# TimoLassmann/tagdust

Measured on AMD Instinct MI355X. Metric: reads/s (150 bp, 8-barcode arch), higher is better.
Workload: dtype f32

## Files before the change

include/tagdust_hip.h:

```cpp
#ifndef TAGDUST_HIP_H
#define TAGDUST_HIP_H

#include <stddef.h>
#include <stdint.h>

#ifdef __cplusplus
extern "C" {
#endif

#define TD_OK   0
#define TD_FAIL 1

#define TD_MAX_SEGMENTS 64
#define TD_MAX_HMMS     127
#define TD_LOGSUM_SIZE  16000

#define TD_MODE_GET_LABEL 1
#define TD_MODE_GET_PROB  4
#define TD_MODE_ARCH_COMP 5
#define TD_MODE_RNA_DUST  6

#define TD_EXTRACT_SUCCESS                    0
#define TD_EXTRACT_FAIL_ARCHITECTURE_MISMATCH 1
#define TD_EXTRACT_FAIL_READ_TOO_SHORT        2
// ... 39 lines not shown
	int32_t read_type;
	int32_t barcode;
	int32_t fingerprint;
} td_read_result;

int  td_ctx_create(int device, td_ctx** out);
void td_ctx_destroy(td_ctx* ctx);
const char* td_last_error(const td_ctx* ctx);

const float* td_logsum_table(void);

int td_model_upload(td_ctx* ctx, const td_model_desc* model);
int td_set_option(td_ctx* ctx, const char* name, int32_t value);
int td_get_option(td_ctx* ctx, const char* name, int32_t* value);
int64_t td_spec_source(const td_model_desc* model, char* buf, int64_t cap);
int td_spec_prune_info(const td_model_desc* model, int32_t lcap, float* tab, float* z, int32_t* n_seg, int32_t* sfx_first);
int td_spec_restart_info(const td_model_desc* model, int32_t lcap, float* tab, int32_t* restart);
#define TD_PROBE_READS     256
#define TD_PROBE_THRESHOLD 3.0f
#define TD_PROBE_MINLEN    16
#define TD_PROBE_DUST      100
#define TD_PROBE_WIN_START 2
#define TD_PROBE_WIN_END   34
int64_t td_spec_probe(const td_model_desc* model, uint8_t* codes, int64_t cap, int64_t* offs);
void td_spec_probe_params(float* threshold, int32_t* minlen, int32_t* dust, int32_t* matchstart, int32_t* matchend);
int td_spec_wait(td_ctx* ctx);
int td_set_artifacts(td_ctx* ctx, const uint8_t* string, const int32_t* s_index, int32_t n_seq,
                     int32_t filter_error, int32_t n_threads);
int td_set_window(td_ctx* ctx, int32_t matchstart, int32_t matchend);
int td_set_batch_window(td_ctx* ctx, int64_t first_read, int64_t total_reads);
// ... 35 lines not shown
```

tagdust_amd/csrc/td_api.hip:

```cpp
#include <math.h>
#include <stdarg.h>
#include <stdlib.h>
#include <string.h>
#include <time.h>
#include <unistd.h>

#include <mutex>
#include <thread>

#include "../../include/tagdust_model.h"
#include "td_ctx.h"
#include "td_rnadust.h"
#include "td_stats.h"

static float g_logsum[TD_LOGSUM_SIZE];
static bool g_logsum_ready = false;
static std::string g_create_error;

static void init_logsum_host()
{
	if (g_logsum_ready) return;
	for (int i = 0; i < TD_LOGSUM_SIZE; i++) g_logsum[i] = (float)log(1.0 + exp((double)-i / (double)1000.0f));
	g_logsum_ready = true;
}
// ... 233 lines not shown
	if (spec_model_uploaded(c) != TD_OK) return TD_FAIL;
	c->have_model = true;
	return TD_OK;
}

extern "C" int td_set_option(td_ctx* c, const char* name, int32_t value)
{
	if (!c || !name) return TD_FAIL;
	if (!strcmp(name, "specialize")) {
		c->spec.specialize = value != 0;
		return TD_OK;
	}
	if (!strcmp(name, "poison_workspace")) { c->poison = value != 0; return TD_OK; }
	if (!strcmp(name, "async_compile")) { c->spec.async_compile = value != 0; return TD_OK; }
	if (!strcmp(name, "spec_probe")) { c->spec.probe = value != 0; return TD_OK; }
	if (!strcmp(name, "compact_egress")) { c->compact_egress = value != 0; return TD_OK; }
	if (!strcmp(name, "stable_input")) {
		if (tickets_outstanding(c)) return fail(c, "td_set_option: stable_input cannot change while tickets are outstanding");
		c->stable_input = value != 0;
		return TD_OK;
	}
	if (!strcmp(name, "length_classes_enabled")) { c->length_classes = value != 0; return TD_OK; }
	if (!strcmp(name, "debug_wait")) { c->debug_wait = value != 0; return TD_OK; }
	if (!strcmp(name, "spec_lsum_limit")) { c->spec.lsum_limit = value > 0 ? (double)value : 1.0e6; return TD_OK; }
	if (!strcmp(name, "rle_cap")) {
		if (value < 0 || value > 127) return fail(c, "td_set_option: rle_cap must be 0 (default) .. 127");
		c->rle_cap_forced = value;
		return TD_OK;
	}
	if (!strcmp(name, "host_threads")) {
// ... 11 lines not shown
		if (tickets_outstanding(c)) return fail(c, "td_set_option: pipeline_depth cannot change while tickets are outstanding");
		c->pipeline_depth = value; c->next_slot = 0;
		return TD_OK;
	}
	return fail(c, "td_set_option: unknown option %s", name);
}

extern "C" int td_get_option(td_ctx* c, const char* name, int32_t* value)
{
	if (!c || !name || !value) return TD_FAIL;
	if (!strcmp(name, "specialize")) { *value = c->spec.specialize; return TD_OK; }
	if (!strcmp(name, "spec_lsum_clamped")) { *value = c->spec.ready && !c->spec.oob; return TD_OK; }
	if (!strcmp(name, "pipeline_depth")) { *value = c->pipeline_depth; return TD_OK; }
	if (!strcmp(name, "async_compile")) { *value = c->spec.async_compile; return TD_OK; }
	if (!strcmp(name, "spec_probe")) { *value = c->spec.probe; return TD_OK; }
	if (!strcmp(name, "spec_state")) { *value = spec_state_now(c); return TD_OK; }
	if (!strcmp(name, "spec_batches_generic")) { *value = c->spec.batches_generic; return TD_OK; }
	if (!strcmp(name, "spec_compiles_started")) { *value = td_spec_compiles_started(); return TD_OK; }
	if (!strcmp(name, "spec_probe_us")) { *value = c->spec.probe_us; return TD_OK; }
	if (!strcmp(name, "host_threads")) { *value = c->host_threads; return TD_OK; }
	if (!strcmp(name, "artifacts_active")) { *value = c->art_n > 0; return TD_OK; }
	if (!strcmp(name, "dust")) { *value = c->dust; return TD_OK; }
	if (!strcmp(name, "length_classes")) { *value = c->slots[c->last_slot].n_big; return TD_OK; }
	if (!strcmp(name, "overlap_decode")) { *value = c->overlap; return TD_OK; }
	if (!strcmp(name, "compact_egress")) { *value = c->compact_egress; return TD_OK; }
	if (!strcmp(name, "stable_input")) { *value = c->stable_input; return TD_OK; }
	if (!strcmp(name, "length_classes_enabled")) { *value = c->length_classes; return TD_OK; }
	if (!strcmp(name, "hw_queues")) { *value = g_hwq_user ? g_hwq_user : (g_hwq_late ? 4 : 8); return TD_OK; }
	if (!strcmp(name, "hw_queues_late")) { *value = g_hwq_late ? 1 : 0; return TD_OK; }
	if (!strcmp(name, "prune_active")) {
// ... 854 lines not shown
```

tagdust_amd/csrc/td_ctx.h:

```cpp
#pragma once
#include <hip/hip_runtime.h>
#include <stdio.h>
#include <memory>
#include <string>
#include <vector>
#include "../../include/tagdust_hip.h"
#include "td_device.h"
#include "td_batch_plan.h"
#include "td_jit.h"
#include "td_stage.h"
#include "td_host_inner.h"
#include "td_census.h"
#include "td_molecules.h"

#define TD_HIDDEN __attribute__((visibility("hidden")))
#define TD_MAX_PIPELINE 4
#define TD_COUNTER_WORDS (TD_NUM_COUNTERS + TD_NUM_DIAG_COUNTERS)

struct TdRoute {
	hipStream_t cs = nullptr;
	hipStream_t aux = nullptr;
	hipStream_t fin = nullptr;
	int wsi = 0;
	bool pipelined = false;
// ... 96 lines not shown
};

struct SpecJob;
struct TdSpecState {
	int specialize = 1;
	bool ready = false;
	hipModule_t mod = nullptr;  hipFunction_t fn = nullptr;
	TdSpecPlan plan;
	bool oob = false;
	bool window = false;
	bool oob_unsafe = false;
	float maxabs = 0.0f;
	int block = 256, waves_per_cu = 8;
	int async_compile = 0;
	int probe = 1;
	int state = 0;
	int batches_generic = 0;
	int probe_us = 0;
	std::shared_ptr<SpecJob> job;
	int job_oob = 0, job_window = 0;
	std::vector<std::shared_ptr<SpecJob>> retired;
	std::string job_err;
	double lsum_limit = 1.0e6;
	int selfcheck_fail = 0;
	float* d_prune = nullptr;   int prune_lcap = 0, prune_stride = 0;
	bool prune_live = false;
};

TD_HIDDEN int default_host_threads();
struct td_ctx {
// ... 143 lines not shown
```

tagdust_amd/csrc/td_jit.h:

```cpp
#pragma once
#include <string>
#include <vector>
#include "../../include/tagdust_hip.h"
#include "td_device.h"

struct TdSpecKnobs {
	int block = 512;
	int min_waves = 4;
	int lsum_oob = 1;
	int rt_min = 16;
	int groupcols = 18;
	int groupcols_fwd = 12;
	int prune = 1;
	int prune_sfx = 1;
	int restart = -1;
	int firstseg = -1;
	int trie_sh = 2;
	int profile = 0;
	int prune_stats = -1;
	std::string extra_opts;
};
TdSpecKnobs td_spec_knobs(void);

#define TD_PRUNE_TABLES 16
#define TD_PRUNE_RESTART_MAX 4

struct TdSpecPlan {
	TdSpecKnobs k;
	int S = 0, H = 0, C = 0;
	std::vector<int> col_off, hmm_off;
	std::vector<int> group, group_f;
	std::vector<int> pure_last, drop_m;
	std::vector<int> bw_off;
	int64_t halves = 0;
	std::vector<int> rt, rt_b;
	std::vector<int> base;
// ... 19 lines not shown
```

tagdust_amd/csrc/td_jit.hip:

```cpp
#include <hip/hip_runtime.h>
#include <hip/hiprtc.h>
#include <math.h>
#include <stdio.h>
#include <string.h>
#include <stdlib.h>

#include <atomic>
#include <map>
#include <mutex>
#include <string>
#include <vector>

#include "../../include/tagdust_hip.h"
#include "td_device.h"
#include <unistd.h>
#include <sys/stat.h>
#include <sys/types.h>
#include "td_embedded_src.h"
#include "td_jit.h"

static std::string flit(float v)
{
	if (isinf(v)) return v < 0 ? "(-__builtin_inff())" : "__builtin_inff()";
	if (v != v) return "__builtin_nanf(\"\")";
// ... 9 lines not shown
	auto flag = [](const char* name, int unset) -> int { const char* e = getenv(name); return e ? atoi(e) != 0 : unset; };
	if (const int v = num("TD_SPEC_BLOCK", 0); v >= 64 && v <= 1024 && v % 64 == 0) k.block = v;
	if (const int v = num("TD_SPEC_MINWAVES", 0); v >= 1 && v <= 8) k.min_waves = v;
	if (const int v = num("TD_SPEC_GROUPCOLS", 0); v > 0) k.groupcols = v;
	k.groupcols_fwd = num("TD_SPEC_GROUPCOLS_FWD", k.groupcols_fwd);
	k.rt_min = num("TD_SPEC_RT_MIN", k.rt_min);
	k.trie_sh = num("TD_SPEC_TRIE_SH", k.trie_sh);
	k.profile = num("TD_SPEC_PROFILE", k.profile);
	k.lsum_oob = flag("TD_SPEC_LSUM_OOB", k.lsum_oob);
	k.prune = flag("TD_SPEC_PRUNE", k.prune);
	k.prune_sfx = flag("TD_SPEC_PRUNE_SFX", k.prune_sfx);
	k.restart = flag("TD_SPEC_RESTART", k.restart);
	k.firstseg = flag("TD_SPEC_FIRSTSEG", k.firstseg);
	k.prune_stats = flag("TD_SPEC_PRUNE_STATS", k.prune_stats);
	if (const char* e = getenv("TD_SPEC_EXTRA_OPTS")) k.extra_opts = e;
	return k;
}

namespace {
int pure_last(const td_model_desc* m, int j, int col_off)
{
	for (int f = 0; f < m->n_hmm[j]; f++) {
		const int q = col_off + f * m->n_col[j] + m->n_col[j] - 1;
		if (!(m->trans[q * 9 + 4] == -INFINITY) || !(m->trans[q * 9 + 3] == -INFINITY)) return 0;
	}
	return 1;
}

int rt_prefix(const td_model_desc* m, int j, int col_off, int* base , float* hi, float* lo, float* nv, int min_hmms)
{
	const int n = m->n_hmm[j], nc = m->n_col[j];
	if (n < min_hmms) return 0;
// ... 309 lines not shown

int td_spec_compile(const td_model_desc* m, const TdSpecPlan& p, int lsum_oob, int window, std::vector<char>& code, std::string& log,
                    uint64_t* key_out, bool key_only)
{
	const std::string src = td_spec_full_source(m, p, lsum_oob, window);
	std::vector<const char*> opts = { "--offload-arch=gfx950", "-O3", "-std=c++17", "-ffp-contract=off", "-fno-fast-math",
	                                  "-fno-slp-vectorize", "-mllvm", "-disable-machine-licm" };
	std::vector<std::string> extra;
	{
		std::string cur;
		for (const char* c = p.k.extra_opts.c_str();; c++) {
			if (*c == ' ' || *c == 0) { if (!cur.empty()) extra.push_back(cur); cur.clear(); if (!*c) break; }
			else cur += *c;
		}
	}
	for (const std::string& o : extra) opts.push_back(o.c_str());
	std::string keytext = src;
	for (const char* o : opts) keytext += std::string(" ") + o;
	{
		int major = 0, minor = 0, rt = 0;
		(void)hiprtcVersion(&major, &minor);
		(void)hipRuntimeGetVersion(&rt);
		keytext += " hiprtc " + std::to_string(major) + "." + std::to_string(minor) + " runtime " + std::to_string(rt);
	}
	const uint64_t key = fnv1a(keytext);
	if (key_out) *key_out = key;
	if (key_only) return TD_OK;
	std::string cache_file;
	const std::string dir = td_spec_cache_dir();
	if (!dir.empty()) {
		char name[64];
// ... 78 lines not shown

extern "C" int td_spec_restart_info(const td_model_desc* model, int32_t lcap, float* tab, int32_t* restart)
{
	if (!model || lcap < 1) return -1;
	const TdSpecPlan p = td_spec_plan(model, td_spec_knobs());
	if (restart) *restart = p.restart;
	if (tab) {
		std::vector<float> t;
		if (p.prune_segs > 0 || p.sfx_first < p.S) td_spec_prune_tables(model, p, lcap, lcap + 8, t);
		else t.assign((size_t)TD_PRUNE_TABLES * (size_t)(lcap + 8), -3.0e38f);
		memcpy(tab, t.data() + (size_t)8 * (size_t)(lcap + 8), (size_t)8 * (size_t)(lcap + 8) * sizeof(float));
	}
	return 0;
}

extern "C" int64_t td_spec_source(const td_model_desc* model, char* buf, int64_t cap)
{
	if (!model) return -1;
	const TdSpecPlan p = td_spec_plan(model, td_spec_knobs());
	const std::string src = td_spec_full_source(model, p, p.k.lsum_oob, 0);
	if (buf && cap > 0) {
		const size_t n = src.size() < (size_t)(cap - 1) ? src.size() : (size_t)(cap - 1);
		memcpy(buf, src.data(), n);
		buf[n] = '\0';
	}
	return (int64_t)src.size();
}
```

tagdust_amd/csrc/td_spec_host.hip:

```cpp
#include <stdlib.h>
#include <algorithm>
#include <cmath>
#include <condition_variable>
#include <map>
#include <mutex>
#include <thread>

#include "td_ctx.h"

struct SpecJob {
	uint64_t key = 0;
	ModelCopy model;
	TdSpecPlan plan;
	int lsum_oob = 0, window = 0;
	std::mutex mu;
	std::condition_variable cv;
	bool done = false;
	int rc = TD_FAIL;
	std::vector<char> code;
	std::string log;
	std::thread th;
	void run()
	{
		std::vector<char> out;
// ... 131 lines not shown
	pc.soa_a = d + o_outa; pc.soa_b = d + o_outb; pc.soa_stride = ol.soa_stride;
	pc.keep_a = ka.out_keep; pc.keep_b = sa.out_keep; pc.labels_a = ka.out_labels; pc.labels_b = sa.out_labels;
	pc.counters_a = cnt_a; pc.counters_b = cnt_b;
	pc.out = (int32_t*)(d + o_cmp);
	HIPCHK(c, td_probe_compare(pc, st));
	int32_t out[1 + 2 * (TD_PROBE_READS / TD_WAVE + 1)];
	HIPCHK(c, hipMemcpyAsync(out, d + o_cmp, sizeof out, hipMemcpyDeviceToHost, st));
	HIPCHK(c, hipStreamSynchronize(st));
	c->spec.prune_lcap = 0; c->spec.prune_live = false;
	v = ProbeVerdict();
	v.mismatches = out[0];
	for (int w = 0; w <= n_tiles && v.read < 0; w++) if (out[1 + 2 * w] >= 0) { v.read = out[1 + 2 * w]; v.field = out[2 + 2 * w]; }
	return TD_OK;
}

static int load_spec_kernel(td_ctx* c, int lsum_oob, int window = -1);
static int start_spec_job(td_ctx* c, int lsum_oob, int window);

static int install_spec_kernel(td_ctx* c, const std::vector<char>& code, uint64_t key, int lsum_oob, int window, bool background)
{
	TdSpecState& sp = c->spec;
	if (spec_unload(c) != TD_OK) return TD_FAIL;
	HIPCHK(c, hipModuleLoadData(&sp.mod, code.data()));
	HIPCHK(c, hipModuleGetFunction(&sp.fn, sp.mod, "td_spec_kernel"));
	{
		static const float g[] = { 0.0f, 0.0005f, 0.001f, 1.0f, 15.699f, 15.6999f, 15.7f, 15.7001f, 16.639f, 16.64f, 16.7f, 100.0f, 1.0e5f, 1.0e6f };
		std::vector<float> pairs;
		for (float base : { 0.0f, -3.25f, -700.0f }) {
			for (float d : g) { pairs.push_back(base); pairs.push_back(base - d); pairs.push_back(base - d); pairs.push_back(base); }
			pairs.push_back(base); pairs.push_back(-INFINITY); pairs.push_back(-INFINITY); pairs.push_back(base);
		}
		pairs.push_back(-INFINITY); pairs.push_back(-INFINITY);
		const int n_pairs = (int)(pairs.size() / 2);
		hipFunction_t chk = nullptr;
// ... 28 lines not shown
		ProbeVerdict v;
		bool known = false;
		{
			std::lock_guard<std::mutex> lk(g_probe_mu);
			auto it = g_probe_verdicts.find({ key, c->device });
			if (it != g_probe_verdicts.end()) { v = it->second; known = true; }
		}
		if (!known) {
			const double t0 = wall_ms();
			if (probe_spec_kernel(c, window, v) != TD_OK) return TD_FAIL;
			sp.probe_us = (int)((wall_ms() - t0) * 1000.0);
			std::lock_guard<std::mutex> lk(g_probe_mu);
			g_probe_verdicts[{ key, c->device }] = v;
		}
		if (v.mismatches != 0) {
			fprintf(stderr, "tagdust_hip: PROBE REJECTED the specialised kernel %016llx on device %d: %d of %d probe reads differ from the generic "
			        "kernel, first at read %d, field %s%s.  This context decodes with the generic kernel: correct, about ten times slower.\n",
			        (unsigned long long)key, c->device, v.mismatches, TD_PROBE_READS, v.read, probe_field_name(v.field), known ? " (verdict of an earlier load)" : "");
			if (spec_unload(c) != TD_OK) return TD_FAIL;
			sp.state = 4;
			return TD_OK;
		}
	}
	sp.ready = true; sp.window = window != 0; sp.oob = lsum_oob != 0;
	sp.state = 3;
	return TD_OK;
}

static int load_spec_kernel(td_ctx* c, int lsum_oob, int window)
{
	if (window < 0) window = c->match_len > 0;
	if (spec_unload(c) != TD_OK) return TD_FAIL;
	std::vector<char> code;
	std::string log;
	uint64_t key = 0;
	if (td_spec_compile(&c->model.d, c->spec.plan, lsum_oob, window, code, log, &key) != TD_OK) {
		c->spec.state = 5;
		return fail(c, "td_model_upload: specialised kernel did not compile: %.400s", log.c_str());
	}
	return install_spec_kernel(c, code, key, lsum_oob, window, false);
}

static int start_spec_job(td_ctx* c, int lsum_oob, int window)
{
	std::vector<char> none;
	std::string log;
	uint64_t key = 0;
	(void)td_spec_compile(&c->model.d, c->spec.plan, lsum_oob, window, none, log, &key, true);
	static std::once_flag at_exit_once;
	std::call_once(at_exit_once, [] { (void)atexit(wait_for_all_spec_jobs); });
	std::shared_ptr<SpecJob> job;
	{
		std::lock_guard<std::mutex> lk(g_jobs_mu);
		for (auto it = g_jobs.begin(); it != g_jobs.end();) { if (it->second.expired()) it = g_jobs.erase(it); else ++it; }
		auto it = g_jobs.find(key);
		if (it != g_jobs.end()) job = it->second.lock();
		if (!job) {
			job = std::make_shared<SpecJob>();
			job->key = key; job->model.assign(&c->model.d); job->plan = c->spec.plan; job->lsum_oob = lsum_oob; job->window = window;
			SpecJob* raw = job.get();
			job->th = std::thread([raw] { raw->run(); });
			g_jobs[key] = job;
		}
	}
	c->spec.job = job; c->spec.job_oob = lsum_oob; c->spec.job_window = window;
	c->spec.state = 1;
	return TD_OK;
}

int spec_handover(td_ctx* c, bool block)
{
	if (!c->spec.job) return c->spec.state == 5 && !c->spec.job_err.empty() ? fail(c, "%s", c->spec.job_err.c_str()) : TD_OK;
	if (!block && !c->spec.job->finished()) return TD_OK;
	c->spec.job->wait();
	const std::shared_ptr<SpecJob> job = std::move(c->spec.job);
	if (job->rc != TD_OK) {
		c->spec.state = 5;
		(void)fail(c, "td_model_upload: specialised kernel did not compile (background compile): %.400s", job->log.c_str());
		c->spec.job_err = c->err;
		return TD_FAIL;
	}
	c->spec.state = 2;
	HIPCHK(c, hipSetDevice(c->device));
	HIPCHK(c, sync_compute(c));
	return install_spec_kernel(c, job->code, job->key, c->spec.job_oob, c->spec.job_window, true);
}

extern "C" int td_spec_wait(td_ctx* c)
{
	if (!c) return TD_FAIL;
	while (c->spec.job) if (spec_handover(c, true) != TD_OK) return TD_FAIL;
	return spec_handover(c, false);
}

int spec_state_now(td_ctx* c) { return c->spec.job ? (c->spec.job->finished() ? 2 : 1) : c->spec.state; }
void spec_retire_jobs(td_ctx* c, bool wait)
{
	if (c->spec.job) { c->spec.retired.push_back(c->spec.job); c->spec.job.reset(); }
	if (wait) { for (auto& j : c->spec.retired) j->wait(); c->spec.retired.clear(); return; }
	for (size_t k = 0; k < c->spec.retired.size();) { if (c->spec.retired[k]->finished()) c->spec.retired.erase(c->spec.retired.begin() + (long)k); else k++; }
// ... 19 lines not shown

int spec_model_uploaded(td_ctx* c)
{
	TdSpecState& sp = c->spec;
	if (spec_unload(c) != TD_OK) return TD_FAIL;
	sp.prune_lcap = 0; sp.prune_live = false;
	sp.state = 0; sp.batches_generic = 0; sp.probe_us = 0;
	if (!sp.specialize) return TD_OK;
	const td_model_desc* m = &c->model.d;
	float mx = 0.0f;
	auto scan = [&](const float* v, size_t n) { for (size_t i = 0; i < n; i++) if (std::isfinite(v[i]) && fabsf(v[i]) > mx) mx = fabsf(v[i]); };
	scan(m->trans, (size_t)m->C * 9); scan(m->eM, (size_t)m->C * 5); scan(m->eI, (size_t)m->C * 5);
	scan(m->sM, m->C); scan(m->sI, m->C); scan(m->skip, m->S); scan(m->bg, 5);
	sp.maxabs = mx;
	sp.plan = td_spec_plan(m, td_spec_knobs());
	sp.block = sp.plan.k.block;
	const int wpb = sp.block / TD_WAVE;
	const int blocks_per_cu = std::min(2, std::max(1, 32 / wpb));
	sp.waves_per_cu = std::min(blocks_per_cu * wpb, 4 * sp.plan.k.min_waves);
	const int oob = sp.oob_unsafe ? 0 : sp.plan.k.lsum_oob;
	return sp.async_compile ? start_spec_job(c, oob, c->match_len > 0) : load_spec_kernel(c, oob);
}
```

tagdust_amd/csrc/td_spec_kernel.inc:

```

#ifndef TDS_BLOCK
#define TDS_BLOCK 512
#endif
#ifndef TDS_MIN_WAVES
#define TDS_MIN_WAVES 4
#endif
#define TDS_REG_H 32
#define TDS_WPB (TDS_BLOCK / TD_WAVE)
#define NEG_INF (-__builtin_inff())
#define DEV __device__ __forceinline__

#define MODE_GET_LABEL 1
#define MODE_ARCH_COMP 5
#define OUT_SUCCESS 0
#define OUT_ARCH_MISMATCH 1
#define OUT_TOO_SHORT 2
#define OUT_BAR_FINGER_NOT_FOUND 3
#define OUT_MATCHES_ARTIFACTS 5
#define OUT_LOW_COMPLEXITY 6
#define N_OUTCOME_SLOTS 8
#define TDS_DIAG(k) (N_OUTCOME_SLOTS + 256 + ((k) - 192))

#ifndef TDS_LSUM_OOB
#define TDS_LSUM_OOB 1
#endif
#if TDS_LSUM_OOB
#define TDS_TABLE_N 16640
#else
#define TDS_TABLE_N (TD_LOGSUM_LIVE + 4)
#endif
__shared__ float g_T[TDS_TABLE_N];

DEV float lsum(float a, float b)
{
#if TDS_LSUM_OOB
	const float t = __builtin_fabsf(a - b) * 4000.0f;
	int idx;
	asm("v_cvt_i32_f32 %0, %1" : "=v"(idx) : "v"(t));
	const float tv = *(const float*)((const char*)g_T + ((unsigned)idx & ~3u));
	return fmaxf(a, b) + tv;
#else
	const float mx = fmaxf(a, b);
	const float dc = fminf(mx - fminf(a, b), 15.7f);
	return mx + g_T[(int)(dc * 1000.0f)];
#endif
}

struct SV { float v; bool z; };
DEV SV sv(float v) { SV r; r.v = v; r.z = false; return r; }
DEV SV sv_none() { SV r; r.v = NEG_INF; r.z = true; return r; }
#define LIVE(v) ((v) != NEG_INF)
DEV SV addc(const SV a, const float c) { SV r; r.z = a.z || !LIVE(c); r.v = r.z ? NEG_INF : a.v + c; return r; }
DEV SV addv(const SV a, const float x) { SV r; r.z = a.z; r.v = a.z ? NEG_INF : a.v + x; return r; }
DEV SV subv(const SV a, const float x) { SV r; r.z = a.z; r.v = a.z ? NEG_INF : a.v - x; return r; }
DEV SV lsum(const SV a, const SV b) { if (a.z) return b; if (b.z) return a; return sv(lsum(a.v, b.v)); }

DEV void lsum2(SV& a0, const SV b0, SV& a1, const SV b1)
{
#if TDS_LSUM_OOB
	if (!a0.z && !b0.z && !a1.z && !b1.z) {
		const float t0 = __builtin_fabsf(a0.v - b0.v) * 4000.0f, t1 = __builtin_fabsf(a1.v - b1.v) * 4000.0f;
		int i0, i1;
		asm("v_cvt_i32_f32 %0, %1" : "=v"(i0) : "v"(t0));
		asm("v_cvt_i32_f32 %0, %1" : "=v"(i1) : "v"(t1));
		const float m0 = fmaxf(a0.v, b0.v), m1 = fmaxf(a1.v, b1.v);
		const float v0 = *(const float*)((const char*)g_T + ((unsigned)i0 & ~3u));
		const float v1 = *(const float*)((const char*)g_T + ((unsigned)i1 & ~3u));
		__builtin_amdgcn_sched_barrier(0);
		a0 = sv(m0 + v0);
		a1 = sv(m1 + v1);
		return;
	}
#endif
	a0 = lsum(a0, b0);
	a1 = lsum(a1, b1);
}

struct SI { float lo, hi; bool z; };
DEV SI si(float lo, float hi) { SI r; r.lo = lo; r.hi = hi; r.z = false; return r; }
DEV SI si(float v) { return si(v, v); }
DEV SI si_none() { SI r; r.lo = NEG_INF; r.hi = NEG_INF; r.z = true; return r; }
DEV SI addc(const SI a, const float c) { SI r; r.z = a.z || !LIVE(c); r.lo = r.z ? NEG_INF : a.lo + c; r.hi = r.z ? NEG_INF : a.hi + c; return r; }
DEV SI addv(const SI a, const float x) { SI r; r.z = a.z; r.lo = a.z ? NEG_INF : a.lo + x; r.hi = a.z ? NEG_INF : a.hi + x; return r; }
DEV float lsum_term(const float d)
{
#if TDS_LSUM_OOB
	const float t = d * 4000.0f;
	int idx;
	asm("v_cvt_i32_f32 %0, %1" : "=v"(idx) : "v"(t));
	return *(const float*)((const char*)g_T + ((unsigned)idx & ~3u));
#else
	return g_T[(int)(fminf(d, 15.7f) * 1000.0f)];
#endif
}
DEV SI lsum(const SI a, const SI b)
{
	if (a.z) return b;
	if (b.z) return a;
	const float dmin = fmaxf(fmaxf(a.lo - b.hi, b.lo - a.hi), 0.0f);
	const float dmax = fmaxf(a.hi - b.lo, b.hi - a.lo);
	return si(fmaxf(a.lo, b.lo) + lsum_term(dmax), fmaxf(a.hi, b.hi) + lsum_term(dmin));
}
DEV bool same(const SI a) { return a.lo == a.hi || (!(a.lo > NEG_INF) && !(a.hi > NEG_INF)); }

typedef float f32x4 __attribute__((ext_vector_type(4)));
// ... 355 lines not shown
#undef EM
}

template <int J, bool RT, int GC>
DEV void stair_dispatch(const int gc, const int fa, float (&Mlo)[kNCol[J]], float (&Mhi)[kNCol[J]], float (&Ilo)[kNCol[J]], float (&Ihi)[kNCol[J]],
                        const float Pn, const BaseMask& kc, const int c, const BaseMask& kx, const int xi)
{
	if constexpr (kNCol[J] > TDS_STAIR_STATIC_COLS) {
		stair_step<J, RT, -2>(gc, fa, Mlo, Mhi, Ilo, Ihi, Pn, kc, c, kx, xi);
	} else if constexpr (GC >= -1) {
		if (gc == GC) stair_step<J, RT, GC>(gc, fa, Mlo, Mhi, Ilo, Ihi, Pn, kc, c, kx, xi);
		else stair_dispatch<J, RT, GC - 1>(gc, fa, Mlo, Mhi, Ilo, Ihi, Pn, kc, c, kx, xi);
	}
}

template <int J, bool RT>
DEV void bwd_stair(const Wv& w, const uint8_t* __restrict__ codes, const float* __restrict__ P, const int fa, const int p_hi, const int p_lo)
{
	constexpr int NC = kNCol[J];
	constexpr int K = NC - 1;
	constexpr bool p_init = (J == TD_S - 1);
#define PBW(pos) (p_init ? (((pos) == w.len + 1) ? 0.0f : NEG_INF) : P[(pos) * TD_WAVE + w.lane])
	const float h = w.hb[(p_hi + 1) * TD_WAVE + w.lane];
	float Mlo[NC], Mhi[NC], Ilo[NC], Ihi[NC];
#pragma unroll
	for (int g = 0; g < NC; g++) { Mlo[g] = NEG_INF; Ilo[g] = NEG_INF; Mhi[g] = h; Ihi[g] = h; }
	int gc = K;
	int c = codes[(p_hi + 1) * TD_WAVE + w.lane];
	float Pn = PBW(p_hi + 1);
	int xi_n = codes[p_hi * TD_WAVE + w.lane];
	float Pi_n = PBW(p_hi);
	int i = p_hi;
// ... 21 lines not shown
	}
	close_check(p_hi - p_lo); close_check(p_hi - p_lo);
	if (gc >= 0) w.bad |= 32;
	if (TDS_PRUNE_STATS && w.lane == 0) {
		const int st = closed_at >= 0 ? closed_at : p_hi - p_lo;
		atomicAdd(&w.stats[TDS_DIAG(196)], (unsigned long long)st); atomicAdd(&w.stats[TDS_DIAG(197)], 1ull);
		atomicMax(&w.stats[TDS_DIAG(193)], (unsigned long long)st);
	}
	float* rs = w.rs + (int64_t)(kColOff[J] + fa * NC) * 2 * TD_WAVE + w.lane;
#pragma unroll
	for (int g = 0; g < NC; g++) { rs[(2 * g) * TD_WAVE] = Mlo[g]; rs[(2 * g + 1) * TD_WAVE] = Ilo[g]; }
#undef PBW
}

template <int J, int F>
DEV void bwd_stair_rest(const Wv& w, const uint8_t* __restrict__ codes, const float* __restrict__ P, const int p_hi, const int p_lo)
{
	if constexpr (F < kNHmm[J]) {
		bwd_stair<J, false>(w, codes, P, F, p_hi, p_lo);
		bwd_stair_rest<J, F + 1>(w, codes, P, p_hi, p_lo);
	}
}

#define TDS_BWD_BOUNDS(d, pos) { const int k_ = w.len - (pos); wc_q[d] = w.wc[k_ >= 1 ? k_ - 1 : 0]; if (skip_live) wd_q[d] = w.wd[k_ >= 0 ? k_ : 0]; }
#define TDS_BWD_STEP(SPILL_, WANT_CS_) \
		const int xi = xi_q[d_]; \
		const bool tailb = sfx_nb && i < w.sstopS; \
		const float Pi = tailb ? NEG_INF : Pi_q[d_]; \
		if (tailb) Pn = NEG_INF; \
		SV cs; cs.v = cs_q[d_]; cs.z = RT ? false : first; \
		{ \
// ... 170 lines not shown
DEV void fold_first_rest(const Wv& w, const int x1, const BaseMask& kx, const float Pi, SV& cs)
{
	if constexpr (F < kNHmm[J]) {
		fold_first_hmm<J, F, false>(w, F, x1, kx, Pi, cs);
		fold_first_rest<J, F + 1>(w, x1, kx, Pi, cs);
	}
}
template <int J>
DEV void bwd_fold_first(const Wv& w, const uint8_t* __restrict__ codes, const float* __restrict__ P, float* __restrict__ Cs)
{
	if (w.len < 1) return;
	const int x1 = codes[1 * TD_WAVE + w.lane];
	const BaseMask kx = mk_mask(x1);
	constexpr bool p_init = (J == TD_S - 1);
	const float Pi = p_init ? ((1 == w.len + 1) ? 0.0f : NEG_INF) : P[1 * TD_WAVE + w.lane];
	SV cs; cs.v = NEG_INF; cs.z = false;
	if constexpr (kRt[J] > 0) { for (int f = 0; f < kRt[J]; f++) fold_first_hmm<J, 0, true>(w, f, x1, kx, Pi, cs); }
	fold_first_rest<J, kRt[J]>(w, x1, kx, Pi, cs);
	Cs[1 * TD_WAVE + w.lane] = cs.v;
}

template <int J, int F0>
DEV void bwd_groups(const Wv& w, const uint8_t* __restrict__ codes, const float* __restrict__ P,
                    float* __restrict__ Cs, uint8_t* __restrict__ BW)
{
	if constexpr (TDS_RESTART && F0 == 0 && J < kPruneSegs) {
		if (w.rb_on) {
			const int p_lo = w.cutS + J * (w.rW + 1), p_hi = p_lo + w.rW;
			bwd_stair_bounds<J>(w, p_hi, p_hi);
			if constexpr (kRtB[J] > 0) { for (int f = 0; f < kRtB[J]; f++) bwd_stair<J, true>(w, codes, P, f, p_hi, p_lo); }
			bwd_stair_rest<J, kRtB[J]>(w, codes, P, p_hi, p_lo);
		}
	}
	if constexpr (F0 == 0 && kRt[J] > 0) {
		if constexpr (kTrieOn && J == 0) {
			for (int f0 = 0; f0 < kTrieNShare * kGroup[J]; f0 += kGroup[J]) bwd_group<J, kGroup[J], true, kTrieSH>(w, codes, P, Cs, BW, f0);
			for (int f0 = kTrieNShare * kGroup[J]; f0 < kRt[J]; f0 += kGroup[J]) bwd_group<J, kGroup[J], true>(w, codes, P, Cs, BW, f0);
		} else {
			for (int f0 = 0; f0 < kRt[J]; f0 += kGroup[J]) bwd_group<J, kGroup[J], true>(w, codes, P, Cs, BW, f0);
		}
		bwd_groups<J, kRt[J]>(w, codes, P, Cs, BW);
	} else if constexpr (F0 < kNHmm[J]) {
		constexpr int NF = cmin(kGroup[J], kNHmm[J] - F0);
		bwd_group<J, NF, false>(w, codes, P, Cs, BW, F0);
		bwd_groups<J, F0 + NF>(w, codes, P, Cs, BW);
	} else if constexpr (kTrieOn && J == 0) {
		bwd_fold_first<J>(w, codes, P, Cs);
	}
}

template <int J>
DEV void bwd_segments(const Wv& w, const uint8_t* __restrict__ codes, float* __restrict__ SB, int rowlen,
                      uint8_t* __restrict__ BW)
{
	if constexpr (J >= 0) {
		bwd_groups<J, 0>(w, codes, SB + (int64_t)(J + 1) * rowlen, SB + (int64_t)J * rowlen, BW);
		if (TDS_PROFILE == 2 && J < 8) { const long long t_ = (long long)__builtin_readcyclecounter(); if (w.lane == 0) atomicAdd(&w.stats[TDS_DIAG(208 + J)], (unsigned long long)(t_ - *w.tprof)); *w.tprof = t_; }
		bwd_segments<J - 1>(w, codes, SB, rowlen, BW);
	}
}

DEV float post_prob(float lp)
{
	float p = 0.0f;
	if (lp > -103.98f) p = (float)exp((double)lp);
	return p;
}
// ... 90 lines not shown
	}
}

template <int J, int GC>
DEV void fstair_dispatch(const int gc, float (&Mlo)[kNCol[J]], float (&Mhi)[kNCol[J]], float (&Ilo)[kNCol[J]], float (&Ihi)[kNCol[J]], const float Pm, const BaseMask& kc)
{
	if constexpr (kNCol[J] > TDS_STAIR_STATIC_COLS) {
		fstair_step<J, -2>(gc, Mlo, Mhi, Ilo, Ihi, Pm, kc);
	} else if constexpr (GC <= kNCol[J]) {
		if (gc == GC) fstair_step<J, GC>(gc, Mlo, Mhi, Ilo, Ihi, Pm, kc);
		else fstair_dispatch<J, GC + 1>(gc, Mlo, Mhi, Ilo, Ihi, Pm, kc);
	}
}

template <int J>
DEV void fwd_stair(const Wv& w, const uint8_t* __restrict__ codes, const float* __restrict__ P, const int q_lo, const int q_hi)
{
	constexpr int NC = kNCol[J];
	float hi0 = NEG_INF;
	{
		const float* gf = w.ptab + (int64_t)(12 + J - kSfxFirst) * w.pstride;
		const int t = q_lo - 1;
		for (int k0 = 1; k0 <= t; k0 += 8) {
			float pr[8];
#pragma unroll
			for (int u = 0; u < 8; u++) { const int k = k0 + u; pr[u] = w.pr[((k <= t) ? t - k : 0) * TD_WAVE + w.lane]; }
			__builtin_amdgcn_sched_barrier(0);
#pragma unroll
			for (int u = 0; u < 8; u++) { const int k = k0 + u; if (k <= t) hi0 = fmaxf(hi0, uload(gf, k) + pr[u]); }
		}
		hi0 = fminf(hi0 + (__logf((float)(t > 1 ? t : 1)) + 0.02f), w.fbs[t]);
// ... 276 lines not shown
		Pm = Pi;
	};
	{
		constexpr bool cs_late = TDS_LATE_CS && (J == TD_S - 1) && !((J == kPruneSegs && kPruneSegs > 0) && skip_live);
		auto step = [&](auto dtag, const int i) __attribute__((always_inline)) { step_cs(dtag, IC<1>{}, i); };
		auto step_nocs = [&](auto dtag, const int i) __attribute__((always_inline)) { step_cs(dtag, IC<0>{}, i); };
		int base = i0;
		if constexpr (cs_late) {
			const int i_cs = (w.tmin < iend) ? w.tmin : iend;
			for (; base + PD - 1 < i_cs; base += PD) ring_block<PD, 0>(step_nocs, base);
		}
		for (; base + PD - 1 <= iend; base += PD) ring_block<PD, 0>(step, base);
		ring_rest<PD, 0>(step, base, iend);
	}
	if (J < kPruneSegs && iend < w.tmax) {
		if (kMaskDP && !own_sum && w.lane == 0) {
#pragma unroll
			for (int f = 0; f < NF; f++)
				for (int wd = ((iend - 1) >> 5) + 1; wd < w.nwm; wd++) w.pmask[(kHmmOff[J] + f0 + f) * w.nwm + wd] = 0u;
		}
		if (kNHmm[J] > 1 && w.len > iend) {
#pragma unroll
			for (int f = 0; f < NF; f++) if (!(tot[f] >= TDS_PRUNE_TT)) w.bad |= 4;
		}
	}
	if (kNHmm[J] > 1) {
#pragma unroll
		for (int f = 0; f < NF; f++) TOTAL[(kHmmOff[J] + f0 + f) * TD_WAVE + w.lane] = tot[f];
	}
#undef EM
#undef PBR
#undef BWROW
#undef TDS_FWD_FILL
}

template <int J, int F0>
DEV void fwd_groups(const Wv& w, const uint8_t* __restrict__ codes, const float* __restrict__ P,
                    float* __restrict__ Cs, const float* __restrict__ PB, const uint8_t* __restrict__ BW,
                    float* __restrict__ DP, float* __restrict__ TOTAL, const float b)
{
	if constexpr (TDS_RESTART && F0 == 0 && J >= kSfxFirst) {
		if (w.rf_on) {
			const int q_hi = w.sstop - (TD_S - 1 - J) * (w.rWf + 1);
			fwd_stair<J>(w, codes, P, q_hi - w.rWf, q_hi);
		}
	}
	if constexpr (F0 == 0 && kRt[J] > 0) {
		for (int f0 = 0; f0 < kRt[J]; f0 += kGroupF[J]) fwd_group<J, kGroupF[J], true>(w, codes, P, Cs, PB, BW, DP, TOTAL, b, f0);
		fwd_groups<J, kRt[J]>(w, codes, P, Cs, PB, BW, DP, TOTAL, b);
	} else if constexpr (F0 < kNHmm[J]) {
		constexpr int NF = cmin(kGroupF[J], kNHmm[J] - F0);
		fwd_group<J, NF, false>(w, codes, P, Cs, PB, BW, DP, TOTAL, b, F0);
		fwd_groups<J, F0 + NF>(w, codes, P, Cs, PB, BW, DP, TOTAL, b);
	}
}

template <int J>
DEV void fwd_segments(const Wv& w, const uint8_t* __restrict__ codes, float* __restrict__ SF, const float* __restrict__ SB,
                      int rowlen, const uint8_t* __restrict__ BW, float* __restrict__ DP, float* __restrict__ TOTAL, const float b)
{
	if constexpr (J < TD_S) {
		fwd_groups<J, 0>(w, codes, SF + (int64_t)J * rowlen, SF + (int64_t)(J + 1) * rowlen, SB + (int64_t)(J + 1) * rowlen,
		                 BW, DP, TOTAL, b);
		if (TDS_PROFILE == 2 && J < 8) { const long long t_ = (long long)__builtin_readcyclecounter(); if (w.lane == 0) atomicAdd(&w.stats[TDS_DIAG(216 + J)], (unsigned long long)(t_ - *w.tprof)); *w.tprof = t_; }
		fwd_segments<J + 1>(w, codes, SF, SB, rowlen, BW, DP, TOTAL, b);
	}
}

constexpr bool path_word_trivial(int k)
{
	for (int b = 0; b < 4; b++) {
		const int v = kFirstN + 4 * k + b;
		if (v < TD_H && (kPredFirst[v] != 0 || kPredOff2[v + 1] != kPredOff2[v])) return false;
// ... 947 lines not shown
```

tagdust_amd/lib.py:

```python
import ctypes as C
import os

import numpy as np

HERE = os.path.dirname(os.path.abspath(__file__))
LIB_PATH = os.environ.get("TD_LIB_PATH", os.path.join(HERE, "libtagdust_hip.so"))

MODE_GET_LABEL = 1
MODE_GET_PROB = 4
MODE_ARCH_COMP = 5
MODE_RNA_DUST = 6
NUM_OUTCOME_SLOTS = 8
NUM_BARCODE_BINS = 256
NUM_COUNTERS = NUM_OUTCOME_SLOTS + NUM_BARCODE_BINS
NUM_DIAG_COUNTERS = 64

ABI_SYMBOLS = [
    "td_ctx_create", "td_ctx_destroy", "td_last_error", "td_logsum_table", "td_model_upload", "td_set_params",
    "td_batch_upload", "td_batch_upload_ascii", "td_run", "td_sync", "td_batch_download", "td_counts_reset",
    "td_counts_get", "td_diag_get", "td_counts_device_ptr", "td_last_kernel_ms", "td_timeline_origin", "td_last_kernel_times", "td_batch_info", "td_set_option", "td_get_option", "td_set_artifacts", "td_spec_source", "td_spec_prune_info", "td_spec_restart_info",
    "td_spec_probe", "td_spec_probe_params", "td_spec_wait",
    "td_submit", "td_wait", "td_host_alloc", "td_host_free", "td_set_batch_window", "td_set_window", "td_arch_scores",
    "td_artifact_hits_get",
]
MULTI_ABI_SYMBOLS = ["td_shard_bounds", "td_count_outcomes", "td_multi_create", "td_multi_destroy", "td_multi_last_error",
                     "td_multi_size", "td_multi_ctx", "td_multi_model_upload", "td_multi_set_params", "td_multi_set_window", "td_multi_set_artifacts",
                     "td_multi_decode", "td_multi_counts", "td_multi_counts_reset", "td_multi_uses_rccl", "td_bind_host_to_device", "td_host_halves_bench",
                     "td_multi_artifact_hits"]
IO_ABI_SYMBOLS = ["td_io_last_error", "td_reads_parse", "td_reads_free", "td_writer_open", "td_writer_write", "td_writer_close",
                  "td_fasta_parse", "td_fasta_free", "td_stream_run", "td_stream_survey", "td_stream_run_multi", "td_stream_run_multi_hits", "td_stream_release",
                  "td_format_q", "td_fingerprint_text", "td_writer_set_fingerprint_text"]
MODEL_ABI_SYMBOLS = ["td_arch_parse", "td_arch_free", "td_sequence_stats", "td_sequence_stats_window", "td_model_build", "td_model_tables_free",
                     "td_calibration_emit", "td_calibration_select", "td_calibration_free", "td_estimate_threshold",
                     "td_compare_architectures", "td_simreads", "td_text_free", "td_sequence_stats_limit",
                     "td_sequence_stats_device"]
# ... 84 lines not shown
    lib.td_ctx_create.argtypes = [C.c_int, C.POINTER(C.c_void_p)]
    lib.td_ctx_destroy.argtypes = [C.c_void_p]
    lib.td_ctx_destroy.restype = None
    lib.td_last_error.argtypes = [C.c_void_p]
    lib.td_last_error.restype = C.c_char_p
    lib.td_logsum_table.restype = C.POINTER(C.c_float)
    lib.td_model_upload.argtypes = [C.c_void_p, C.POINTER(_ModelDesc)]
    lib.td_set_params.argtypes = [C.c_void_p, C.c_float, C.c_int32, C.c_int32]
    lib.td_set_option.argtypes = [C.c_void_p, C.c_char_p, C.c_int32]
    if hasattr(lib, "td_set_artifacts"):
        lib.td_set_artifacts.argtypes = [C.c_void_p, C.c_void_p, C.c_void_p, C.c_int32, C.c_int32, C.c_int32]
    if hasattr(lib, "td_get_option"):
        lib.td_get_option.argtypes = [C.c_void_p, C.c_char_p, C.POINTER(C.c_int32)]
    lib.td_spec_source.argtypes = [C.POINTER(_ModelDesc), C.c_char_p, C.c_int64]
    lib.td_spec_source.restype = C.c_int64
    lib.td_spec_prune_info.argtypes = [C.POINTER(_ModelDesc), C.c_int32, C.c_void_p, C.POINTER(C.c_float), C.POINTER(C.c_int32), C.POINTER(C.c_int32)]
    lib.td_batch_upload.argtypes = [C.c_void_p, C.c_void_p, C.c_void_p, C.c_int64]
    lib.td_batch_upload_ascii.argtypes = [C.c_void_p, C.c_void_p, C.c_void_p, C.c_int64]
    lib.td_run.argtypes = [C.c_void_p, C.c_int]
    lib.td_sync.argtypes = [C.c_void_p]
    lib.td_batch_download.argtypes = [C.c_void_p, C.c_void_p, C.c_void_p, C.c_void_p]
    lib.td_submit.argtypes = [C.c_void_p, C.c_void_p, C.c_int32, C.c_void_p, C.c_int64, C.c_int, C.c_void_p, C.c_void_p, C.c_void_p,
                              C.POINTER(C.c_int64)]
    lib.td_wait.argtypes = [C.c_void_p, C.c_int64]
    lib.td_host_alloc.argtypes = [C.c_size_t]
    lib.td_host_alloc.restype = C.c_void_p
    lib.td_host_free.argtypes = [C.c_void_p]
    lib.td_host_free.restype = None
    lib.td_set_batch_window.argtypes = [C.c_void_p, C.c_int64, C.c_int64]
    lib.td_set_window.argtypes = [C.c_void_p, C.c_int32, C.c_int32]
# ... 930 lines not shown
def stream_release():
    lib = load_library()
    lib.td_stream_release.restype = None
    lib.td_stream_release()


def spec_source(md):
    lib = load_library()
    d, keep = make_model_desc(md)
    n = lib.td_spec_source(C.byref(d), None, 0)
    buf = C.create_string_buffer(int(n) + 1)
    lib.td_spec_source(C.byref(d), buf, int(n) + 1)
    return buf.value.decode()


PROBE_READS = 256


def spec_probe(md):
    lib = load_library()
    lib.td_spec_probe.argtypes = [C.POINTER(_ModelDesc), C.c_void_p, C.c_int64, C.c_void_p]
    lib.td_spec_probe.restype = C.c_int64
    d, keep = make_model_desc(md)
    offs = np.zeros(PROBE_READS + 1, np.int64)
    n = int(lib.td_spec_probe(C.byref(d), None, 0, offs.ctypes.data))
    if n < 0:
        raise TdError("td_spec_probe: bad model description")
    codes = np.zeros(n, np.uint8)
    lib.td_spec_probe(C.byref(d), codes.ctypes.data, n, None)
    return codes, offs
# ... 517 lines not shown
```

Before: 80.27 million.

## Build specialised kernel with iterative-ILP scheduler, falling back to default on probe mismatch

```diff
diff --git a/include/tagdust_hip.h b/include/tagdust_hip.h
--- a/include/tagdust_hip.h
+++ b/include/tagdust_hip.h
@@ -77,6 +77,7 @@
 int td_set_option(td_ctx* ctx, const char* name, int32_t value);
 int td_get_option(td_ctx* ctx, const char* name, int32_t* value);
 int64_t td_spec_source(const td_model_desc* model, char* buf, int64_t cap);
+int td_spec_key(const td_model_desc* model, const char* sched, uint64_t* key);
 int td_spec_prune_info(const td_model_desc* model, int32_t lcap, float* tab, float* z, int32_t* n_seg, int32_t* sfx_first);
 int td_spec_restart_info(const td_model_desc* model, int32_t lcap, float* tab, int32_t* restart);
 #define TD_PROBE_READS     256
diff --git a/tagdust_amd/csrc/td_api.hip b/tagdust_amd/csrc/td_api.hip
--- a/tagdust_amd/csrc/td_api.hip
+++ b/tagdust_amd/csrc/td_api.hip
@@ -271,6 +271,11 @@
 	if (!strcmp(name, "poison_workspace")) { c->poison = value != 0; return TD_OK; }
 	if (!strcmp(name, "async_compile")) { c->spec.async_compile = value != 0; return TD_OK; }
 	if (!strcmp(name, "spec_probe")) { c->spec.probe = value != 0; return TD_OK; }
+	if (!strcmp(name, "spec_sched")) {
+		if (value != 0 && value != TD_SCHED_DEFAULT && value != TD_SCHED_ILP) return fail(c, "td_set_option: spec_sched must be 0 (TD_SPEC_SCHED or the built-in choice), 1 (default) or 2 (iterative-ilp)");
+		c->spec.sched = value;
+		return TD_OK;
+	}
 	if (!strcmp(name, "compact_egress")) { c->compact_egress = value != 0; return TD_OK; }
 	if (!strcmp(name, "stable_input")) {
 		if (tickets_outstanding(c)) return fail(c, "td_set_option: stable_input cannot change while tickets are outstanding");
@@ -312,6 +317,8 @@
 	if (!strcmp(name, "pipeline_depth")) { *value = c->pipeline_depth; return TD_OK; }
 	if (!strcmp(name, "async_compile")) { *value = c->spec.async_compile; return TD_OK; }
 	if (!strcmp(name, "spec_probe")) { *value = c->spec.probe; return TD_OK; }
+	if (!strcmp(name, "spec_sched")) { *value = c->spec.sched; return TD_OK; }
+	if (!strcmp(name, "spec_sched_active")) { *value = c->spec.ready ? c->spec.sched_active : 0; return TD_OK; }
 	if (!strcmp(name, "spec_state")) { *value = spec_state_now(c); return TD_OK; }
 	if (!strcmp(name, "spec_batches_generic")) { *value = c->spec.batches_generic; return TD_OK; }
 	if (!strcmp(name, "spec_compiles_started")) { *value = td_spec_compiles_started(); return TD_OK; }
diff --git a/tagdust_amd/csrc/td_ctx.h b/tagdust_amd/csrc/td_ctx.h
--- a/tagdust_amd/csrc/td_ctx.h
+++ b/tagdust_amd/csrc/td_ctx.h
@@ -134,6 +134,9 @@
 	int block = 256, waves_per_cu = 8;
 	int async_compile = 0;
 	int probe = 1;
+	int sched = 0;
+	int sched_active = 0;
+	int job_sched = 0;
 	int state = 0;
 	int batches_generic = 0;
 	int probe_us = 0;
diff --git a/tagdust_amd/csrc/td_jit.h b/tagdust_amd/csrc/td_jit.h
--- a/tagdust_amd/csrc/td_jit.h
+++ b/tagdust_amd/csrc/td_jit.h
@@ -3,6 +3,9 @@
 #include <vector>
 #include "../../include/tagdust_hip.h"
 #include "td_device.h"
+
+#define TD_SCHED_DEFAULT 1
+#define TD_SCHED_ILP 2
 
 struct TdSpecKnobs {
 	int block = 512;
@@ -19,7 +22,11 @@
 	int profile = 0;
 	int prune_stats = -1;
 	std::string extra_opts;
+	int sched = TD_SCHED_ILP;
+	int extra_opts_sched = 0;
 };
+int td_spec_sched_parse(const char* name);
+const char* td_spec_sched_name(int sched);
 TdSpecKnobs td_spec_knobs(void);
 
 #define TD_PRUNE_TABLES 16
diff --git a/tagdust_amd/csrc/td_jit.hip b/tagdust_amd/csrc/td_jit.hip
--- a/tagdust_amd/csrc/td_jit.hip
+++ b/tagdust_amd/csrc/td_jit.hip
@@ -47,8 +47,17 @@
 	k.firstseg = flag("TD_SPEC_FIRSTSEG", k.firstseg);
 	k.prune_stats = flag("TD_SPEC_PRUNE_STATS", k.prune_stats);
 	if (const char* e = getenv("TD_SPEC_EXTRA_OPTS")) k.extra_opts = e;
+	if (const int v = td_spec_sched_parse(getenv("TD_SPEC_SCHED"))) k.sched = v;
+	k.extra_opts_sched = td_spec_sched_parse(getenv("TD_SPEC_EXTRA_OPTS_SCHED"));
 	return k;
 }
+
+int td_spec_sched_parse(const char* name)
+{
+	if (!name) return 0;
+	return !strcmp(name, "default") ? TD_SCHED_DEFAULT : !strcmp(name, "iterative-ilp") ? TD_SCHED_ILP : 0;
+}
+const char* td_spec_sched_name(int sched) { return sched == TD_SCHED_ILP ? "iterative-ilp" : "default"; }
 
 namespace {
 int pure_last(const td_model_desc* m, int j, int col_off)
@@ -388,7 +397,9 @@
 			else cur += *c;
 		}
 	}
-	for (const std::string& o : extra) opts.push_back(o.c_str());
+	if (p.k.sched == TD_SCHED_ILP) { opts.push_back("-mllvm"); opts.push_back("-amdgpu-sched-strategy=iterative-ilp"); }
+	if (!p.k.extra_opts_sched || p.k.extra_opts_sched == p.k.sched)
+		for (const std::string& o : extra) opts.push_back(o.c_str());
 	std::string keytext = src;
 	for (const char* o : opts) keytext += std::string(" ") + o;
 	{
@@ -497,6 +508,17 @@
 	return 0;
 }
 
+extern "C" int td_spec_key(const td_model_desc* model, const char* sched, uint64_t* key)
+{
+	if (!model || !key) return -1;
+	TdSpecKnobs k = td_spec_knobs();
+	if (sched) { const int v = td_spec_sched_parse(sched); if (!v) return -1; k.sched = v; }
+	const TdSpecPlan p = td_spec_plan(model, k);
+	std::vector<char> none;
+	std::string log;
+	return td_spec_compile(model, p, p.k.lsum_oob, 0, none, log, key, true) == TD_OK ? 0 : -1;
+}
+
 extern "C" int64_t td_spec_source(const td_model_desc* model, char* buf, int64_t cap)
 {
 	if (!model) return -1;
diff --git a/tagdust_amd/csrc/td_spec_host.hip b/tagdust_amd/csrc/td_spec_host.hip
--- a/tagdust_amd/csrc/td_spec_host.hip
+++ b/tagdust_amd/csrc/td_spec_host.hip
@@ -169,10 +169,10 @@
 	return TD_OK;
 }
 
-static int load_spec_kernel(td_ctx* c, int lsum_oob, int window = -1);
-static int start_spec_job(td_ctx* c, int lsum_oob, int window);
-
-static int install_spec_kernel(td_ctx* c, const std::vector<char>& code, uint64_t key, int lsum_oob, int window, bool background)
+static int load_spec_kernel(td_ctx* c, int lsum_oob, int window = -1, int sched = 0);
+static int start_spec_job(td_ctx* c, int lsum_oob, int window, int sched = 0);
+
+static int install_spec_kernel(td_ctx* c, const std::vector<char>& code, uint64_t key, int lsum_oob, int window, int sched, bool background)
 {
 	TdSpecState& sp = c->spec;
 	if (spec_unload(c) != TD_OK) return TD_FAIL;
@@ -231,39 +231,48 @@
 			g_probe_verdicts[{ key, c->device }] = v;
 		}
 		if (v.mismatches != 0) {
-			fprintf(stderr, "tagdust_hip: PROBE REJECTED the specialised kernel %016llx on device %d: %d of %d probe reads differ from the generic "
-			        "kernel, first at read %d, field %s%s.  This context decodes with the generic kernel: correct, about ten times slower.\n",
-			        (unsigned long long)key, c->device, v.mismatches, TD_PROBE_READS, v.read, probe_field_name(v.field), known ? " (verdict of an earlier load)" : "");
+			const bool retry = sched == TD_SCHED_ILP;
+			fprintf(stderr, "tagdust_hip: PROBE REJECTED the specialised kernel %016llx (machine scheduler: %s) on device %d: %d of %d probe reads differ "
+			        "from the generic kernel, first at read %d, field %s%s.  %s\n",
+			        (unsigned long long)key, td_spec_sched_name(sched), c->device, v.mismatches, TD_PROBE_READS, v.read, probe_field_name(v.field),
+			        known ? " (verdict of an earlier load)" : "",
+			        retry ? "The same source is built with the default scheduler instead."
+			              : "This context decodes with the generic kernel: correct, about ten times slower.");
 			if (spec_unload(c) != TD_OK) return TD_FAIL;
+			if (retry) return background ? start_spec_job(c, lsum_oob, window, TD_SCHED_DEFAULT) : load_spec_kernel(c, lsum_oob, window, TD_SCHED_DEFAULT);
 			sp.state = 4;
 			return TD_OK;
 		}
 	}
-	sp.ready = true; sp.window = window != 0; sp.oob = lsum_oob != 0;
+	sp.ready = true; sp.window = window != 0; sp.oob = lsum_oob != 0; sp.sched_active = sched;
 	sp.state = 3;
 	return TD_OK;
 }
 
-static int load_spec_kernel(td_ctx* c, int lsum_oob, int window)
+static int load_spec_kernel(td_ctx* c, int lsum_oob, int window, int sched)
 {
 	if (window < 0) window = c->match_len > 0;
 	if (spec_unload(c) != TD_OK) return TD_FAIL;
 	std::vector<char> code;
 	std::string log;
 	uint64_t key = 0;
-	if (td_spec_compile(&c->model.d, c->spec.plan, lsum_oob, window, code, log, &key) != TD_OK) {
+	TdSpecPlan plan = c->spec.plan;
+	if (sched) plan.k.sched = sched; else sched = plan.k.sched;
+	if (td_spec_compile(&c->model.d, plan, lsum_oob, window, code, log, &key) != TD_OK) {
 		c->spec.state = 5;
 		return fail(c, "td_model_upload: specialised kernel did not compile: %.400s", log.c_str());
 	}
-	return install_spec_kernel(c, code, key, lsum_oob, window, false);
-}
-
-static int start_spec_job(td_ctx* c, int lsum_oob, int window)
+	return install_spec_kernel(c, code, key, lsum_oob, window, sched, false);
+}
+
+static int start_spec_job(td_ctx* c, int lsum_oob, int window, int sched)
 {
 	std::vector<char> none;
 	std::string log;
 	uint64_t key = 0;
-	(void)td_spec_compile(&c->model.d, c->spec.plan, lsum_oob, window, none, log, &key, true);
+	TdSpecPlan plan = c->spec.plan;
+	if (sched) plan.k.sched = sched; else sched = plan.k.sched;
+	(void)td_spec_compile(&c->model.d, plan, lsum_oob, window, none, log, &key, true);
 	static std::once_flag at_exit_once;
 	std::call_once(at_exit_once, [] { (void)atexit(wait_for_all_spec_jobs); });
 	std::shared_ptr<SpecJob> job;
@@ -274,13 +283,13 @@
 		if (it != g_jobs.end()) job = it->second.lock();
 		if (!job) {
 			job = std::make_shared<SpecJob>();
-			job->key = key; job->model.assign(&c->model.d); job->plan = c->spec.plan; job->lsum_oob = lsum_oob; job->window = window;
+			job->key = key; job->model.assign(&c->model.d); job->plan = plan; job->lsum_oob = lsum_oob; job->window = window;
 			SpecJob* raw = job.get();
 			job->th = std::thread([raw] { raw->run(); });
 			g_jobs[key] = job;
 		}
 	}
-	c->spec.job = job; c->spec.job_oob = lsum_oob; c->spec.job_window = window;
+	c->spec.job = job; c->spec.job_oob = lsum_oob; c->spec.job_window = window; c->spec.job_sched = sched;
 	c->spec.state = 1;
 	return TD_OK;
 }
@@ -300,7 +309,7 @@
 	c->spec.state = 2;
 	HIPCHK(c, hipSetDevice(c->device));
 	HIPCHK(c, sync_compute(c));
-	return install_spec_kernel(c, job->code, job->key, c->spec.job_oob, c->spec.job_window, true);
+	return install_spec_kernel(c, job->code, job->key, c->spec.job_oob, c->spec.job_window, c->spec.job_sched, true);
 }
 
 extern "C" int td_spec_wait(td_ctx* c)
@@ -350,6 +359,7 @@
 	scan(m->sM, m->C); scan(m->sI, m->C); scan(m->skip, m->S); scan(m->bg, 5);
 	sp.maxabs = mx;
 	sp.plan = td_spec_plan(m, td_spec_knobs());
+	if (sp.sched) sp.plan.k.sched = sp.sched;
 	sp.block = sp.plan.k.block;
 	const int wpb = sp.block / TD_WAVE;
 	const int blocks_per_cu = std::min(2, std::max(1, 32 / wpb));
diff --git a/tagdust_amd/csrc/td_spec_kernel.inc b/tagdust_amd/csrc/td_spec_kernel.inc
--- a/tagdust_amd/csrc/td_spec_kernel.inc
+++ b/tagdust_amd/csrc/td_spec_kernel.inc
@@ -30,6 +30,14 @@
 #define TDS_TABLE_N (TD_LOGSUM_LIVE + 4)
 #endif
 __shared__ float g_T[TDS_TABLE_N];
+#if TDS_LSUM_OOB
+DEV float lds_gather(const unsigned off)
+{
+	typedef const __attribute__((address_space(3))) float* lds_cf;
+	const unsigned table = (unsigned)(__UINTPTR_TYPE__)(lds_cf)g_T;
+	return *(lds_cf)(__UINTPTR_TYPE__)(table + off);
+}
+#endif
 
 DEV float lsum(float a, float b)
 {
@@ -37,7 +45,7 @@
 	const float t = __builtin_fabsf(a - b) * 4000.0f;
 	int idx;
 	asm("v_cvt_i32_f32 %0, %1" : "=v"(idx) : "v"(t));
-	const float tv = *(const float*)((const char*)g_T + ((unsigned)idx & ~3u));
+	const float tv = lds_gather((unsigned)idx & ~3u);
 	return fmaxf(a, b) + tv;
 #else
 	const float mx = fmaxf(a, b);
@@ -64,8 +72,8 @@
 		asm("v_cvt_i32_f32 %0, %1" : "=v"(i0) : "v"(t0));
 		asm("v_cvt_i32_f32 %0, %1" : "=v"(i1) : "v"(t1));
 		const float m0 = fmaxf(a0.v, b0.v), m1 = fmaxf(a1.v, b1.v);
-		const float v0 = *(const float*)((const char*)g_T + ((unsigned)i0 & ~3u));
-		const float v1 = *(const float*)((const char*)g_T + ((unsigned)i1 & ~3u));
+		const float v0 = lds_gather((unsigned)i0 & ~3u);
+		const float v1 = lds_gather((unsigned)i1 & ~3u);
 		__builtin_amdgcn_sched_barrier(0);
 		a0 = sv(m0 + v0);
 		a1 = sv(m1 + v1);
@@ -88,7 +96,7 @@
 	const float t = d * 4000.0f;
 	int idx;
 	asm("v_cvt_i32_f32 %0, %1" : "=v"(idx) : "v"(t));
-	return *(const float*)((const char*)g_T + ((unsigned)idx & ~3u));
+	return lds_gather((unsigned)idx & ~3u);
 #else
 	return g_T[(int)(fminf(d, 15.7f) * 1000.0f)];
 #endif
@@ -474,8 +482,9 @@
 	}
 }
 
+
 template <int J, bool RT>
-DEV void bwd_stair(const Wv& w, const uint8_t* __restrict__ codes, const float* __restrict__ P, const int fa, const int p_hi, const int p_lo)
+DEV void bwd_stair(const Wv& w, const uint8_t* __restrict__ codes, const float* P, const int fa, const int p_hi, const int p_lo)
 {
 	constexpr int NC = kNCol[J];
 	constexpr int K = NC - 1;
@@ -527,7 +536,7 @@
 }
 
 template <int J, int F>
-DEV void bwd_stair_rest(const Wv& w, const uint8_t* __restrict__ codes, const float* __restrict__ P, const int p_hi, const int p_lo)
+DEV void bwd_stair_rest(const Wv& w, const uint8_t* __restrict__ codes, const float* P, const int p_hi, const int p_lo)
 {
 	if constexpr (F < kNHmm[J]) {
 		bwd_stair<J, false>(w, codes, P, F, p_hi, p_lo);
@@ -728,15 +737,18 @@
 	const BaseMask kx = mk_mask(x1);
 	constexpr bool p_init = (J == TD_S - 1);
 	const float Pi = p_init ? ((1 == w.len + 1) ? 0.0f : NEG_INF) : P[1 * TD_WAVE + w.lane];
-	SV cs; cs.v = NEG_INF; cs.z = false;
-	if constexpr (kRt[J] > 0) { for (int f = 0; f < kRt[J]; f++) fold_first_hmm<J, 0, true>(w, f, x1, kx, Pi, cs); }
+	SV cs = sv_none();
+	if constexpr (kRt[J] > 0) {
+		fold_first_hmm<J, 0, true>(w, 0, x1, kx, Pi, cs);
+		for (int f = 1; f < kRt[J]; f++) fold_first_hmm<J, 0, true>(w, f, x1, kx, Pi, cs);
+	}
 	fold_first_rest<J, kRt[J]>(w, x1, kx, Pi, cs);
 	Cs[1 * TD_WAVE + w.lane] = cs.v;
 }
 
 template <int J, int F0>
-DEV void bwd_groups(const Wv& w, const uint8_t* __restrict__ codes, const float* __restrict__ P,
-                    float* __restrict__ Cs, uint8_t* __restrict__ BW)
+DEV void bwd_groups(const Wv& w, const uint8_t* __restrict__ codes, const float* P,
+                    float* Cs, uint8_t* __restrict__ BW)
 {
 	if constexpr (TDS_RESTART && F0 == 0 && J < kPruneSegs) {
 		if (w.rb_on) {
@@ -764,7 +776,7 @@
 }
 
 template <int J>
-DEV void bwd_segments(const Wv& w, const uint8_t* __restrict__ codes, float* __restrict__ SB, int rowlen,
+DEV void bwd_segments(const Wv& w, const uint8_t* __restrict__ codes, float* SB, int rowlen,
                       uint8_t* __restrict__ BW)
 {
 	if constexpr (J >= 0) {
@@ -885,7 +897,7 @@
 }
 
 template <int J>
-DEV void fwd_stair(const Wv& w, const uint8_t* __restrict__ codes, const float* __restrict__ P, const int q_lo, const int q_hi)
+DEV void fwd_stair(const Wv& w, const uint8_t* __restrict__ codes, const float* P, const int q_lo, const int q_hi)
 {
 	constexpr int NC = kNCol[J];
 	float hi0 = NEG_INF;
@@ -1192,7 +1204,7 @@
 		ring_rest<PD, 0>(step, base, iend);
 	}
 	if (J < kPruneSegs && iend < w.tmax) {
-		if (kMaskDP && !own_sum && w.lane == 0) {
+		if (kMaskDP && !own_sum) {
 #pragma unroll
 			for (int f = 0; f < NF; f++)
 				for (int wd = ((iend - 1) >> 5) + 1; wd < w.nwm; wd++) w.pmask[(kHmmOff[J] + f0 + f) * w.nwm + wd] = 0u;
@@ -1213,8 +1225,8 @@
 }
 
 template <int J, int F0>
-DEV void fwd_groups(const Wv& w, const uint8_t* __restrict__ codes, const float* __restrict__ P,
-                    float* __restrict__ Cs, const float* __restrict__ PB, const uint8_t* __restrict__ BW,
+DEV void fwd_groups(const Wv& w, const uint8_t* __restrict__ codes, const float* P,
+                    float* Cs, const float* PB, const uint8_t* __restrict__ BW,
                     float* __restrict__ DP, float* __restrict__ TOTAL, const float b)
 {
 	if constexpr (TDS_RESTART && F0 == 0 && J >= kSfxFirst) {
@@ -1234,7 +1246,7 @@
 }
 
 template <int J>
-DEV void fwd_segments(const Wv& w, const uint8_t* __restrict__ codes, float* __restrict__ SF, const float* __restrict__ SB,
+DEV void fwd_segments(const Wv& w, const uint8_t* __restrict__ codes, float* SF, const float* SB,
                       int rowlen, const uint8_t* __restrict__ BW, float* __restrict__ DP, float* __restrict__ TOTAL, const float b)
 {
 	if constexpr (J < TD_S) {
diff --git a/tagdust_amd/lib.py b/tagdust_amd/lib.py
--- a/tagdust_amd/lib.py
+++ b/tagdust_amd/lib.py
@@ -18,7 +18,7 @@
 ABI_SYMBOLS = [
     "td_ctx_create", "td_ctx_destroy", "td_last_error", "td_logsum_table", "td_model_upload", "td_set_params",
     "td_batch_upload", "td_batch_upload_ascii", "td_run", "td_sync", "td_batch_download", "td_counts_reset",
-    "td_counts_get", "td_diag_get", "td_counts_device_ptr", "td_last_kernel_ms", "td_timeline_origin", "td_last_kernel_times", "td_batch_info", "td_set_option", "td_get_option", "td_set_artifacts", "td_spec_source", "td_spec_prune_info", "td_spec_restart_info",
+    "td_counts_get", "td_diag_get", "td_counts_device_ptr", "td_last_kernel_ms", "td_timeline_origin", "td_last_kernel_times", "td_batch_info", "td_set_option", "td_get_option", "td_set_artifacts", "td_spec_source", "td_spec_key", "td_spec_prune_info", "td_spec_restart_info",
     "td_spec_probe", "td_spec_probe_params", "td_spec_wait",
     "td_submit", "td_wait", "td_host_alloc", "td_host_free", "td_set_batch_window", "td_set_window", "td_arch_scores",
     "td_artifact_hits_get",
@@ -133,6 +133,8 @@
         lib.td_get_option.argtypes = [C.c_void_p, C.c_char_p, C.POINTER(C.c_int32)]
     lib.td_spec_source.argtypes = [C.POINTER(_ModelDesc), C.c_char_p, C.c_int64]
     lib.td_spec_source.restype = C.c_int64
+    if hasattr(lib, "td_spec_key"):
+        lib.td_spec_key.argtypes = [C.POINTER(_ModelDesc), C.c_char_p, C.POINTER(C.c_uint64)]
     lib.td_spec_prune_info.argtypes = [C.POINTER(_ModelDesc), C.c_int32, C.c_void_p, C.POINTER(C.c_float), C.POINTER(C.c_int32), C.POINTER(C.c_int32)]
     lib.td_batch_upload.argtypes = [C.c_void_p, C.c_void_p, C.c_void_p, C.c_int64]
     lib.td_batch_upload_ascii.argtypes = [C.c_void_p, C.c_void_p, C.c_void_p, C.c_int64]
@@ -1093,6 +1095,19 @@
     return buf.value.decode()
 
 
+SCHED_DEFAULT, SCHED_ILP = 1, 2
+SCHED_NAMES = {SCHED_DEFAULT: "default", SCHED_ILP: "iterative-ilp"}
+
+
+def spec_key(md, sched=None):
+    lib = load_library()
+    d, keep = make_model_desc(md)
+    key = C.c_uint64(0)
+    if lib.td_spec_key(C.byref(d), sched.encode() if sched else None, C.byref(key)) != 0:
+        raise ValueError("td_spec_key: unknown scheduler strategy %r" % (sched,))
+    return int(key.value)
+
+
 PROBE_READS = 256
 
 
```

Result: no change. 80.57 million (median of 2 runs) (+0.4%).
